# wasiahmad/context_attentive_ir

Measured on AMD Instinct MI355X. Metric: ranked (query,doc) pairs/sec, higher is better.
Workload: dtype f32; 1 GPU; cars, batch=16 sessions x session_len 7 x 10 candidates, q_len=4, doc_len=64, emb_dim=300, vocab=100000, f32, full-length Zipf ids; macro_batch=8, lanes=4, batches_in_flight=32, hipgraph=True, parallelism=single GPU, world_size=1

## Files before the change

### context_attentive_ir_amd/csrc/lstm_fold.hip

```cpp
#include <type_traits>
#include "split2.hpp"
#include <hip/hip_bf16.h>
#include <string>
#include <algorithm>

namespace nir {

int launch_linear(const float* a, int64_t lda, const int64_t* ids, const float* table, int E, int64_t rows_per_seq,
                  int64_t seq_stride, const float* w, int64_t ldw, const float* bias, const float* bias2, float* c,
                  int64_t ldc, int64_t M, int N, int K, int act, hipStream_t st);

__global__ void fold_permute_kernel(const float* __restrict__ wih, const float* __restrict__ bih, const float* __restrict__ bhh,
                                    int H, int ND, int E, float* __restrict__ wperm, float* __restrict__ bperm) {
    const int64_t i = (int64_t)blockIdx.x * blockDim.x + threadIdx.x;
    const int64_t rows = (int64_t)ND * 4 * H;
    if (i >= rows * E) return;
    const int64_t ro = i / E;
    const int k = (int)(i % E);
    const int gate = (int)(ro & 3), unit = (int)((ro >> 2) % H), dir = (int)((ro >> 2) / H);
    const int64_t ri = (int64_t)dir * 4 * H + (int64_t)gate * H + unit;
    wperm[i] = wih[ri * E + k];
    if (k == 0) bperm[ro] = bih[ri] + bhh[ri];
}

__global__ void iota_i64_kernel(int64_t* __restrict__ out, int64_t n) {
    const int64_t i = (int64_t)blockIdx.x * blockDim.x + threadIdx.x;
    if (i < n) out[i] = i;
}

int launch_fold_permute(const float* w_ih, const float* b_ih, const float* b_hh, int H, int ndir, int E, float* wperm, float* bperm, int64_t* iota, int64_t niota,
                        hipStream_t st) {
    const int64_t n = (int64_t)ndir * 4 * H * E;
    hipLaunchKernelGGL(fold_permute_kernel, dim3((unsigned)((n + 255) / 256)), dim3(256), 0, st, w_ih, b_ih, b_hh, H, ndir, E, wperm, bperm);
    if (iota && niota > 0) hipLaunchKernelGGL(iota_i64_kernel, dim3((unsigned)((niota + 255) / 256)), dim3(256), 0, st, iota, niota);
    NIR_CHECK_LAUNCH("fold_permute_kernel");
    return 0;
}

__global__ void f32_to_bf16_kernel(const float* __restrict__ src, unsigned short* __restrict__ dst, int64_t n) {
    const int64_t i = ((int64_t)blockIdx.x * blockDim.x + threadIdx.x) * 4;
    if (i + 3 < n) {
        const float4 v = *reinterpret_cast<const float4*>(src + i);
        ushort4 o;
        o.x = f2bf(v.x); o.y = f2bf(v.y); o.z = f2bf(v.z); o.w = f2bf(v.w);
        *reinterpret_cast<ushort4*>(dst + i) = o;
    } else {
        for (int64_t j = i; j < n; ++j) dst[j] = f2bf(src[j]);
    }
}

struct LstmPtArgs {
    const void* pt;
    const int64_t* ids;
    const int64_t* lens;
    const float* whh;
    float* out;
    int* err;
    int64_t M, V;
    int T, H, ND;
    int out_f16;
    const void* whh_frag;
    float* act;
    float* cst;
};

template <int G, int NT>
__global__ __launch_bounds__(1024) void lstm16_pt_kernel(LstmPtArgs p) {
    constexpr int SEQ = 16, KP = 16 * G, ZLD = KP + 4;
    constexpr uint32_t OOB = 0x7FFFFFF0u;
    extern __shared__ __attribute__((aligned(16))) float smem[];
    float* z = smem;
    int* lens_s = reinterpret_cast<int*>(z + 2 * SEQ * ZLD);
    int* ids_s = lens_s + SEQ;

    const int tid = threadIdx.x, lane = tid & 63, wave = tid >> 6;
    const int sq = lane & 15, kq = lane >> 4;
    const int dir = blockIdx.y;
    const int64_t m0 = (int64_t)blockIdx.x * SEQ;
    const int H = p.H, T = p.T, H4 = 4 * H;
    const int nvalid = (int)min((int64_t)SEQ, p.M - m0);
    const int OW = p.ND * H;
    const int64_t GW = (int64_t)p.ND * H4;
    const int ntiles = (H + 3) / 4;

    if (tid < SEQ) {
        int l = 0;
        if (tid < nvalid) {
            l = p.lens ? (int)p.lens[m0 + tid] : T;
            l = l < 0 ? 0 : (l > T ? T : l);
        }
        lens_s[tid] = l;
    }
    {
        bool bad = false;
        for (int e = tid; e < SEQ * T; e += 1024) {
            const int s = e / T;
            int64_t id = 0;
            if (s < nvalid) id = p.ids[m0 * T + e];
            if (id < 0 || id >= p.V) { bad = true; id = 0; }
            ids_s[e] = (int)id;
        }
        if (bad && p.err) atomicOr(p.err, 1);
    }
    for (int e = tid; e < 2 * SEQ * ZLD; e += 1024) z[e] = 0.f;
    __syncthreads();
    int tmax = 0;
#pragma unroll
    for (int s2 = 0; s2 < SEQ; ++s2) tmax = max(tmax, lens_s[s2]);
    const int mylen = lens_s[sq];

    float wreg[NT][4 * G];
    float creg[NT], hreg[NT];
    int unit_d[NT];
#pragma unroll
    for (int t = 0; t < NT; ++t) {
        const int tile = NT * wave + t;
        const int unit_a = 4 * tile + (sq >> 2), gate_a = sq & 3;
        const bool av = unit_a < H;
        const float* wr = p.whh + ((int64_t)dir * H4 + (int64_t)gate_a * H + (av ? unit_a : 0)) * H;
#pragma unroll
        for (int q = 0; q < G; ++q)
#pragma unroll
            for (int j = 0; j < 4; ++j) {
                const int k = 16 * q + 4 * kq + j;
                wreg[t][4 * q + j] = wr[k < H ? k : H - 1] * ((av && k < H) ? 1.f : 0.f);
            }
        unit_d[t] = 4 * tile + kq;
        creg[t] = 0.f;
        hreg[t] = 0.f;
    }
    const __amdgpu_buffer_rsrc_t out_rs = __builtin_amdgcn_make_buffer_rsrc(p.out + m0 * T * OW, 0,
                                                                             (int)((uint32_t)nvalid * T * OW * 4u), 0x00020000);
    const float* ptf = reinterpret_cast<const float*>(p.pt) + (int64_t)dir * H4;
    auto load_g = [&](int step, f32x4 (&dst)[NT]) {
        int s_ = min(step, mylen - 1);
        s_ = s_ < 0 ? 0 : s_;
        const int t_ = dir == 0 ? s_ : mylen - 1 - s_;
        const int id = ids_s[sq * T + (t_ < 0 ? 0 : t_)];
        const float* row = ptf + (int64_t)id * GW;
#pragma unroll
        for (int t = 0; t < NT; ++t) {
            const int u = unit_d[t] < H ? unit_d[t] : H - 1;
            dst[t] = *reinterpret_cast<const f32x4*>(row + 4 * u);
        }
    };
    f32x4 gcur[NT], gnext[NT];
    load_g(0, gcur);

    const bool has1 = NT * wave < ntiles;
    const bool has2 = NT > 1 && NT * wave + 1 < ntiles;
    for (int step = 0; step < tmax; ++step) {
        const float* zc = z + (step & 1) * SEQ * ZLD;
        float* zn = z + ((step + 1) & 1) * SEQ * ZLD;
        load_g(step + 1, gnext);
        const bool live = step < mylen;
        const int tt = dir == 0 ? step : mylen - 1 - step;
        auto cell_tile = [&](int t, const f32x4& acc) {
// ... 82 lines not shown
        const bool av = unit_a < H;
        const float* wr = p.whh + ((int64_t)dir * H4 + (int64_t)gate_a * H + (av ? unit_a : 0)) * H;
        const bool vec_ok = (H % 8) == 0 && ((reinterpret_cast<uintptr_t>(wr) & 15) == 0);
        if (vec_ok) {
#pragma unroll
            for (int kb = 0; kb < KB; ++kb) {
                const int k0 = 32 * kb + 8 * kq;
                const int kc = k0 + 8 <= H ? k0 : 0;
                const float4 a = *reinterpret_cast<const float4*>(wr + kc), b = *reinterpret_cast<const float4*>(wr + kc + 4);
                const float m = (av && k0 + 8 <= H) ? 1.f : 0.f;
                wreg[t][kb][0] = (_Float16)(a.x * m); wreg[t][kb][1] = (_Float16)(a.y * m);
                wreg[t][kb][2] = (_Float16)(a.z * m); wreg[t][kb][3] = (_Float16)(a.w * m);
                wreg[t][kb][4] = (_Float16)(b.x * m); wreg[t][kb][5] = (_Float16)(b.y * m);
                wreg[t][kb][6] = (_Float16)(b.z * m); wreg[t][kb][7] = (_Float16)(b.w * m);
                wbad |= !(fmaxf(fmaxf(fmaxf(fabsf(a.x), fabsf(a.y)), fmaxf(fabsf(a.z), fabsf(a.w))),
                                fmaxf(fmaxf(fabsf(b.x), fabsf(b.y)), fmaxf(fabsf(b.z), fabsf(b.w)))) * m < 65504.0f);
            }
        } else {
#pragma unroll
            for (int kb = 0; kb < KB; ++kb)
#pragma unroll
                for (int j = 0; j < 8; ++j) {
                    const int k = 32 * kb + 8 * kq + j;
                    const float w = wr[k < H ? k : H - 1] * ((av && k < H) ? 1.f : 0.f);
                    wreg[t][kb][j] = (_Float16)w;
                    wbad |= !(fabsf(w) < 65504.0f);
                }
        }
        unit_d[t] = 4 * tile + kq;
    }
    if (wbad && p.err) atomicOr(p.err, 2);
    for (int64_t mt = blockIdx.x; mt * SEQ < p.M; mt += gridDim.x) {
        __syncthreads();
        const int64_t m0 = mt * SEQ;
        const int nvalid = (int)min((int64_t)SEQ, p.M - m0);

        if (tid < SEQ) {
            int l = 0;
            if (tid < nvalid) {
                l = p.lens ? (int)p.lens[m0 + tid] : T;
                l = l < 0 ? 0 : (l > T ? T : l);
            }
            lens_s[tid] = l;
        }
        {
            bool bad = false;
            for (int e = tid; e < SEQ * T; e += 1024) {
                const int s = e / T;
                int64_t id = 0;
                if (s < nvalid) id = p.ids[m0 * T + e];
                if (id < 0 || id >= p.V) { bad = true; id = 0; }
                ids_s[e] = (int)id;
            }
            if (bad && p.err) atomicOr(p.err, 1);
        }
        for (int e = tid; e < SEQ * ZLD; e += 1024) reinterpret_cast<unsigned*>(z)[e] = 0u;
        __syncthreads();
        int tmax = 0;
#pragma unroll
        for (int s2 = 0; s2 < SEQ; ++s2) tmax = max(tmax, lens_s[s2]);
        const int mylen = lens_s[sq];

#pragma unroll
        for (int t = 0; t < NT; ++t) creg[t] = 0.f;
        const __amdgpu_buffer_rsrc_t out_rs =
            O16 ? __builtin_amdgcn_make_buffer_rsrc(reinterpret_cast<_Float16*>(p.out) + m0 * T * OW, 0, (int)((uint32_t)nvalid * T * OW * 2u), 0x00020000)
                : __builtin_amdgcn_make_buffer_rsrc(p.out + m0 * T * OW, 0, (int)((uint32_t)nvalid * T * OW * 4u), 0x00020000);
        const int wlen = __builtin_amdgcn_readfirstlane(lens_s[wave & (SEQ - 1)]);
        auto copy_out = [&](int s_, const unsigned short* zsrc) {
            const bool on = s_ >= 0 && s_ < wlen && 2 * lane < H;
            const int tt_ = dir == 0 ? s_ : wlen - 1 - s_;
            const uint32_t v = *reinterpret_cast<const uint32_t*>(zsrc + wave * ZLD + 2 * lane);
            const uint32_t off = on ? (uint32_t)((wave * T + tt_) * OW + dir * H + 2 * lane) * 2u : OOB;
            __builtin_amdgcn_raw_buffer_store_b32(v, out_rs, off, 0, 0);
        };
        const unsigned short* pth = reinterpret_cast<const unsigned short*>(p.pt) + (int64_t)dir * H4;
        auto id_of = [&](int step) {
            int s_ = min(step, mylen - 1);
            s_ = s_ < 0 ? 0 : s_;
            const int t_ = dir == 0 ? s_ : mylen - 1 - s_;
            return ids_s[sq * T + (t_ < 0 ? 0 : t_)];
        };
        auto load_g = [&](int id, uint2 (&dst)[NT]) {
            const unsigned short* row = pth + (int64_t)id * GW;
#pragma unroll
            for (int t = 0; t < NT; ++t) {
                const int u = unit_d[t] < H ? unit_d[t] : H - 1;
                dst[t] = *reinterpret_cast<const uint2*>(row + 4 * u);
            }
        };
        uint2 ga[NT], gb[NT];
        load_g(id_of(0), ga);
#pragma unroll
        for (int t = 0; t < (O16 ? 1 : NT); ++t) __builtin_amdgcn_raw_buffer_store_b32(0u, out_rs, OOB, 0, 0);
        load_g(id_of(1), gb);
#pragma unroll
        for (int t = 0; t < (O16 ? 1 : NT); ++t) __builtin_amdgcn_raw_buffer_store_b32(0u, out_rs, OOB, 0, 0);
        int id_n = id_of(2);

        for (int step = 0; step < tmax; ++step) {
            const unsigned short* zc = z + (step & 1) * SEQ * ZLD;
            unsigned short* zn = z + ((step + 1) & 1) * SEQ * ZLD;
            f32x4 acc[NT];
#pragma unroll
            for (int t = 0; t < NT; ++t) {
                asm volatile("" : "+v"(ga[t].x), "+v"(ga[t].y));
                acc[t] = (f32x4){bf2f((unsigned short)(ga[t].x & 0xFFFFu)), bf2f((unsigned short)(ga[t].x >> 16)),
                                 bf2f((unsigned short)(ga[t].y & 0xFFFFu)), bf2f((unsigned short)(ga[t].y >> 16))};
                ga[t] = gb[t];
            }
            const bool live = step < mylen;
            const int tt = dir == 0 ? step : mylen - 1 - step;
            const unsigned short* zr = zc + sq * ZLD + 8 * kq;
            if (O16) copy_out(step - 1, zc);
#pragma unroll
            for (int kb = 0; kb < KB; ++kb) {
                const f16x8 hb = *reinterpret_cast<const f16x8*>(zr + 32 * kb);
#pragma unroll
                for (int t = 0; t < NT; ++t) acc[t] = __builtin_amdgcn_mfma_f32_16x16x32_f16(wreg[t][kb], hb, acc[t], 0, 0, 0);
                if (kb == 0) {
                    load_g(id_n, gb);
                    id_n = id_of(step + 3);
                }
            }
#pragma unroll
            for (int t = 0; t < NT; ++t) {
                uint32_t off = OOB;
                float hv = 0.f;
                if (NT * wave + t < ntiles) {
                    const bool dv = unit_d[t] < H;
                    float hn;
                    lstm_cell_v(acc[t], creg[t], hn);
                    if (dv) reinterpret_cast<_Float16*>(zn)[sq * ZLD + unit_d[t]] = (_Float16)hn;
                    if (dv && live) off = (uint32_t)((sq * T + tt) * OW + dir * H + unit_d[t]) * 4u;
                    hv = hn;
                }
                if (!O16) __builtin_amdgcn_raw_buffer_store_b32(__float_as_uint(hv), out_rs, off, 0, 0);
            }
            lds_barrier();
        }
        if (O16 && tmax > 0) copy_out(tmax - 1, z + (tmax & 1) * SEQ * ZLD);
        for (int s_ = 0; s_ < nvalid; ++s_) {
            const int64_t ob = (m0 + s_) * T * OW + (int64_t)dir * H;
            for (int t2 = lens_s[s_] + wave; t2 < T; t2 += 16)
                for (int col = lane; col < H; col += 64) {
                    if (O16) reinterpret_cast<_Float16*>(p.out)[ob + (int64_t)t2 * OW + col] = (_Float16)0.f;
                    else p.out[ob + (int64_t)t2 * OW + col] = 0.f;
                }
        }
    }
}


#ifdef NIR_PT_TRACE
__device__ unsigned long long* g_pt_trace_dev;
#define PT_T(var) asm volatile("s_memtime %0\n\ts_waitcnt lgkmcnt(0)" : "=s"(var) :: "memory")
#endif
template <int KB, int NT, int NW, bool H1 = false, bool TR = false>
__global__ __launch_bounds__(64 * NW, NW <= 4 ? 2 : 1) void lstm16_pt_h2_kernel(LstmPtArgs p) {
    static_assert(!TR || !H1, "train-mode stores go with the fp32 output");
    constexpr int NTH = 64 * NW;
    constexpr int SEQ = 16, KP = 32 * KB, ZLD = KP + 8;
    constexpr uint32_t OOB = 0x7FFFFFF0u;
    constexpr bool SWZ = KB == 4;
    constexpr int KBS = SWZ ? 16 : 32;
    auto zoff = [](int s_, int k_) -> int {
        if constexpr (SWZ) {
            const int q_ = (k_ >> 3) & 3, b_ = k_ >> 5;
            return (s_ ^ (8 * (q_ & 1))) * ZLD + (8 * (q_ & 1) + 2 * b_ + (q_ >> 1)) * 8 + (k_ & 7);
        } else {
            return s_ * ZLD + k_;
        }
    };
#ifdef NIR_X_NOPIPE
    constexpr bool PIPE = false;
#else
    constexpr bool PIPE = NT >= 4 && NW == 8;
#endif
    constexpr bool DEFER = NW >= 8;
    const int TP = p.T + 3;
    extern __shared__ __attribute__((aligned(16))) float smem[];
    _Float16* z = reinterpret_cast<_Float16*>(smem);
    int* lens_s = reinterpret_cast<int*>(z + 4 * SEQ * ZLD);
    int* simd_s = lens_s + SEQ;
    int* ids_s = simd_s + 16;

    const int tid = threadIdx.x, lane = tid & 63, wave = tid >> 6;
    const int sq = lane & 15, kq = lane >> 4;
    const int dir = blockIdx.y;
    const int64_t m0 = (int64_t)blockIdx.x * SEQ;
    const int H = p.H, T = p.T, H4 = 4 * H;
    const int nvalid = (int)min((int64_t)SEQ, p.M - m0);
    const int OW = p.ND * H;
    const int64_t GW = (int64_t)p.ND * H4;
    f16x8 w1[NT][KB], w2[NT][KB];
    const bool use_frag = KB == 4 && NT == 4 && NW == 8 && p.whh_frag != nullptr && H == 128;
    if (use_frag) {
        const f16x8* fp = reinterpret_cast<const f16x8*>(p.whh_frag) + ((size_t)(dir * NW + wave) * NT * KB * 2) * 64 + lane;
#pragma unroll
        for (int t = 0; t < NT; ++t)
#pragma unroll
            for (int kb = 0; kb < KB; ++kb) {
                w1[t][kb] = fp[((t * KB + kb) * 2 + 0) * 64];
                w2[t][kb] = fp[((t * KB + kb) * 2 + 1) * 64];
            }
    }
    if (NW > 4 && lane == 0) simd_s[wave] = (int)__builtin_amdgcn_s_getreg(4 | (4 << 6) | (1 << 11));
    if (tid < SEQ) {
        int l = 0;
        if (tid < nvalid) {
            l = p.lens ? (int)p.lens[m0 + tid] : T;
            l = l < 0 ? 0 : (l > T ? T : l);
        }
        lens_s[tid] = l;
    }
    lds_barrier();
    {
        bool bad = false;
        for (int e = tid; e < SEQ * TP; e += NTH) {
            const int s_ = e / TP, k = e - s_ * TP;
            int64_t id = 0;
            if (s_ < nvalid) {
                const int l = lens_s[s_];
                int kk = k < l - 1 ? k : l - 1;
                kk = kk < 0 ? 0 : kk;
                int t_ = dir == 0 ? kk : l - 1 - kk;
                t_ = t_ < 0 ? 0 : t_;
                id = p.ids[(m0 + s_) * T + t_];
                if (k < T) {
                    const int64_t raw = p.ids[(m0 + s_) * T + k];
                    bad |= raw < 0 || raw >= p.V;
                }
            }
            if (id < 0 || id >= p.V) id = 0;
            ids_s[e] = (int)id;
        }
        if (bad && p.err) atomicOr(p.err, 1);
    }
    for (int e = tid; e < 2 * SEQ * ZLD; e += NTH) reinterpret_cast<unsigned*>(z)[e] = 0u;
    lds_barrier();
    int tmax = 0;
#pragma unroll
    for (int s2 = 0; s2 < SEQ; ++s2) tmax = max(tmax, lens_s[s2]);
    const int mylen = lens_s[sq];
    if (NW > 4) {
        const int mine = simd_s[wave];
        int rank = 0;
#pragma unroll
        for (int w2_ = 0; w2_ < NW; ++w2_) rank += (w2_ < wave && simd_s[w2_] == mine) ? 1 : 0;
        rank = __builtin_amdgcn_readfirstlane(rank);
        if (rank == 0) __builtin_amdgcn_s_setprio(3);
        else if (rank == 1) __builtin_amdgcn_s_setprio(2);
        else if (rank == 2) __builtin_amdgcn_s_setprio(1);
        else __builtin_amdgcn_s_setprio(0);
    }

    float creg[NT];
    const int u0 = NT * (4 * wave + kq);
    const bool wave_on = PIPE || NT * 4 * wave < H;
    const bool full = u0 + NT <= H;
    bool wbad = false;
#pragma unroll
    for (int t = 0; t < NT; ++t) {
        if (use_frag) { creg[t] = 0.f; continue; }
        const int unit_a = NT * (4 * wave + (sq >> 2)) + t, gate_a = sq & 3;
        const bool av = unit_a < H;
        const float* wr = p.whh + ((int64_t)dir * H4 + (int64_t)gate_a * H + (av ? unit_a : 0)) * H;
        float wv[KB][8];
        const bool vec_ok = (H % 8) == 0 && ((reinterpret_cast<uintptr_t>(wr) & 15) == 0);
        if (vec_ok) {
#pragma unroll
            for (int kb = 0; kb < KB; ++kb) {
                const int k0 = 32 * kb + 8 * kq;
                const int kc = k0 + 8 <= H ? k0 : 0;
                const float4 a = *reinterpret_cast<const float4*>(wr + kc), b = *reinterpret_cast<const float4*>(wr + kc + 4);
                const float m = (av && k0 + 8 <= H) ? 1.f : 0.f;
                wv[kb][0] = a.x * m; wv[kb][1] = a.y * m; wv[kb][2] = a.z * m; wv[kb][3] = a.w * m;
                wv[kb][4] = b.x * m; wv[kb][5] = b.y * m; wv[kb][6] = b.z * m; wv[kb][7] = b.w * m;
            }
        } else {
#pragma unroll
            for (int kb = 0; kb < KB; ++kb)
#pragma unroll
                for (int j = 0; j < 8; ++j) {
                    const int k = 32 * kb + 8 * kq + j;
                    wv[kb][j] = wr[k < H ? k : H - 1] * ((av && k < H) ? 1.f : 0.f);
                }
        }
#pragma unroll
        for (int kb = 0; kb < KB; ++kb)
#pragma unroll
            for (int j = 0; j < 8; ++j) {
                const float w = wv[kb][j];
                const _Float16 a = split2_hi1_rne(w);
                w1[t][kb][j] = a;
                w2[t][kb][j] = split2_lo1(w, a);
                wbad |= !(fabsf(w) < 32768.0f);
            }
        creg[t] = 0.f;
    }
    if (wbad && p.err) atomicOr(p.err, 2);
    const __amdgpu_buffer_rsrc_t out_rs = H1 ? __builtin_amdgcn_make_buffer_rsrc(reinterpret_cast<_Float16*>(p.out) + m0 * T * OW, 0,
                                                                                  (int)((uint32_t)nvalid * T * OW * 2u), 0x00020000)
                                             : __builtin_amdgcn_make_buffer_rsrc(p.out + m0 * T * OW, 0, (int)((uint32_t)nvalid * T * OW * 4u), 0x00020000);
    const __amdgpu_buffer_rsrc_t act_rs = __builtin_amdgcn_make_buffer_rsrc(TR ? p.act + m0 * T * GW : p.out, 0,
                                                                             TR ? (int)((uint32_t)nvalid * T * (uint32_t)GW * 4u) : 0, 0x00020000);
    const __amdgpu_buffer_rsrc_t cst_rs = __builtin_amdgcn_make_buffer_rsrc(TR ? p.cst + m0 * T * OW : p.out, 0,
                                                                             TR ? (int)((uint32_t)nvalid * T * OW * 4u) : 0, 0x00020000);
    const float* ptf = reinterpret_cast<const float*>(p.pt) + (int64_t)dir * H4;
    const float* pb[NT];
#pragma unroll
    for (int t = 0; t < NT; ++t) pb[t] = ptf + 4 * (u0 + t < H ? u0 + t : H - 1);
    const uint32_t gw = (uint32_t)GW;
    auto load_g = [&](int id, f32x4 (&dst)[NT]) {
#ifdef NIR_X_NOROWS
        return;
#endif
        const uint64_t ro = (uint64_t)(uint32_t)id * gw;
#pragma unroll
        for (int t = 0; t < NT; ++t) dst[t] = *reinterpret_cast<const f32x4*>(pb[t] + ro);
    };
    f32x4 gnext[NT];
    uint32_t hprev[NT];
#pragma unroll
    for (int t = 0; t < NT; ++t) hprev[t] = 0u;
    const bool split = NT == 4 && p.out_f16 == 2;
    uint32_t poff = OOB;
    auto store_prev = [&]() {
#ifdef NIR_X_NOSTORE
        return;
#endif
        if (H1) {
            __builtin_amdgcn_raw_buffer_store_b64((u32x2){hprev[0], hprev[1 % NT]}, out_rs, poff == OOB ? OOB : poff >> 1, 0, 0);
            return;
        }
        if (NT == 4) {
            __builtin_amdgcn_raw_buffer_store_b128((u32x4){hprev[0], hprev[1 % NT], hprev[2 % NT], hprev[3 % NT]}, out_rs, full ? poff : OOB, 0, 0);
        } else if (NT == 2) {
            __builtin_amdgcn_raw_buffer_store_b64((u32x2){hprev[0], hprev[1 % NT]}, out_rs, full ? poff : OOB, 0, 0);
        }
        if ((NT != 4 && NT != 2) || !full) {
#pragma unroll
            for (int t = 0; t < NT; ++t)
                __builtin_amdgcn_raw_buffer_store_b32(hprev[t], out_rs, (u0 + t < H && poff != OOB) ? poff + 4u * t : OOB, 0, 0);
        }
    };
    const int* idp = ids_s + sq * TP;
    load_g(idp[0], gnext);
    int id_n = idp[1];
    uint32_t soff = (uint32_t)(((sq * T + (dir == 0 ? 0 : mylen - 1)) * OW + dir * H + u0) * 4);
    const uint32_t sstep = (uint32_t)(dir == 0 ? OW * 4 : -(OW * 4));
    f32x4 acc[NT], acx[NT];
    float hn[NT] = {};
#ifdef NIR_X_NOGATES
    auto gates = [&](int t) { hn[t] = (acx[t][0] + acc[t][1]) * 1e-3f; };
#else
    float tga[TR ? NT : 1][4];
    auto gates = [&](int t) {
        if constexpr (TR) {
            const f32x4 x = split2_combine(acc[t], acx[t]);
            const float gi = fast_sigmoid(x[0]), gf = fast_sigmoid(x[1]), gg = fast_tanh(x[2]), go = fast_sigmoid(x[3]);
            const float cn = gf * creg[t] + gi * gg;
            creg[t] = cn;
            hn[t] = go * fast_tanh(cn);
            tga[t][0] = gi; tga[t][1] = gf; tga[t][2] = gg; tga[t][3] = go;
        } else {
            lstm_cell_v(split2_combine(acc[t], acx[t]), creg[t], hn[t]);
        }
    };
    uint32_t aoff = (uint32_t)(((int64_t)(sq * T + (dir == 0 ? 0 : mylen - 1)) * GW + dir * H4 + u0) * 4);
    const uint32_t astep = (uint32_t)(dir == 0 ? GW * 4 : -(GW * 4));
#endif
#ifdef NIR_PT_TRACE
    unsigned long long tr_a = 0, tr_b = 0, tr_c = 0, tr_t0 = 0, tr_t1 = 0, tr_t2 = 0, tr_first = 0, tr_l = 0, tr_m = 0;
#endif
    for (int step = 0; step < tmax; ++step) {
#ifdef NIR_PT_TRACE
        { unsigned long long tn; PT_T(tn); if (step > 0) tr_c += tn - tr_t2; else tr_first = tn; tr_t0 = tn; }
#endif
        const _Float16* zc = z + (step & 1) * 2 * SEQ * ZLD;
        _Float16* zn = z + ((step + 1) & 1) * 2 * SEQ * ZLD;
#pragma unroll
        for (int t = 0; t < NT; ++t) {
            acc[t] = gnext[t];
            acx[t] = (f32x4){0.f, 0.f, 0.f, 0.f};
        }
        const bool live = step < mylen;
        const _Float16* zr = zc + zoff(sq, 8 * kq);
        if (!wave_on) {
#ifdef NIR_X_BURST
        } else if constexpr (NT == 4 && NW == 8) {
            f16x8 hh1[KB], hh2[KB];
#pragma unroll
            for (int kb = 0; kb < KB; ++kb) {
                hh1[kb] = *reinterpret_cast<const f16x8*>(zr + KBS * kb);
                hh2[kb] = *reinterpret_cast<const f16x8*>(zr + SEQ * ZLD + KBS * kb);
            }
#pragma unroll
            for (int kb = 0; kb < KB; ++kb) {
#pragma unroll
                for (int t = 0; t < NT; ++t) acc[t] = __builtin_amdgcn_mfma_f32_16x16x32_f16(w1[t][kb], hh1[kb], acc[t], 0, 0, 0);
#pragma unroll
                for (int t = 0; t < NT; ++t) acx[t] = __builtin_amdgcn_mfma_f32_16x16x32_f16(w1[t][kb], hh2[kb], acx[t], 0, 0, 0);
#pragma unroll
                for (int t = 0; t < NT; ++t) acx[t] = __builtin_amdgcn_mfma_f32_16x16x32_f16(w2[t][kb], hh1[kb], acx[t], 0, 0, 0);
                if (kb == 0) {
                    if (DEFER) store_prev();
                    load_g(id_n, gnext);
                    id_n = idp[step + 2];
                }
            }
#ifdef NIR_PT_TRACE
#pragma unroll
            for (int t = 0; t < NT; ++t) asm volatile("" : "+v"(acc[t]), "+v"(acx[t]));
            PT_T(tr_t1); tr_a += tr_t1 - tr_t0;
#endif
#pragma unroll
            for (int t = 0; t < NT; ++t) gates(t);
#endif
        } else if constexpr (!PIPE) {
#pragma unroll
            for (int kb = 0; kb < KB; ++kb) {
                const f16x8 h1 = *reinterpret_cast<const f16x8*>(zr + KBS * kb);
                const f16x8 h2 = *reinterpret_cast<const f16x8*>(zr + SEQ * ZLD + KBS * kb);
#pragma unroll
                for (int t = 0; t < NT; ++t) {
                    acc[t] = __builtin_amdgcn_mfma_f32_16x16x32_f16(w1[t][kb], h1, acc[t], 0, 0, 0);
                    acx[t] = __builtin_amdgcn_mfma_f32_16x16x32_f16(w1[t][kb], h2, acx[t], 0, 0, 0);
                    acx[t] = __builtin_amdgcn_mfma_f32_16x16x32_f16(w2[t][kb], h1, acx[t], 0, 0, 0);
                }
                if (kb == 0) {
                    if (DEFER) store_prev();
                    load_g(id_n, gnext);
                    id_n = idp[step + 2];
                }
            }
#ifdef NIR_PT_TRACE
#pragma unroll
            for (int t = 0; t < NT; ++t) asm volatile("" : "+v"(acc[t]), "+v"(acx[t]));
            PT_T(tr_t1); tr_a += tr_t1 - tr_t0;
#endif
#pragma unroll
            for (int t = 0; t < NT; ++t) gates(t);
        } else {
            f16x8 hh1[KB], hh2[H1 ? 1 : KB];
#pragma unroll
            for (int kb = 0; kb < KB; ++kb) {
                hh1[kb] = *reinterpret_cast<const f16x8*>(zr + KBS * kb);
                if (!H1) hh2[H1 ? 0 : kb] = *reinterpret_cast<const f16x8*>(zr + SEQ * ZLD + KBS * kb);
            }
#ifdef NIR_PT_TRACE
            { unsigned long long tn; PT_T(tn); tr_l += tn - tr_t0; }
#endif
#pragma unroll
            for (int t = 0; t < NT; ++t) {
#pragma unroll
                for (int kb = 0; kb < KB; ++kb) {
                    acc[t] = __builtin_amdgcn_mfma_f32_16x16x32_f16(w1[t][kb], hh1[kb], acc[t], 0, 0, 0);
                    if (!H1) acx[t] = __builtin_amdgcn_mfma_f32_16x16x32_f16(w1[t][kb], hh2[H1 ? 0 : kb], acx[t], 0, 0, 0);
                    acx[t] = __builtin_amdgcn_mfma_f32_16x16x32_f16(w2[t][kb], hh1[kb], acx[t], 0, 0, 0);
                }
                if (t == 0) {
                    if (DEFER) store_prev();
                    load_g(id_n, gnext);
                    id_n = idp[step + 2];
                } else {
#ifdef NIR_PT_TRACE
                    if (t == 1) { asm volatile("" : "+v"(acc[0]), "+v"(acx[0])); unsigned long long tn; PT_T(tn); tr_m += tn - tr_t0; }
#endif
                    gates(t - 1);
#pragma unroll
                    for (int q = 0; q < (H1 ? 2 : 3) * KB; ++q) {
                        __builtin_amdgcn_sched_group_barrier(0x008, 1, 0);
                        __builtin_amdgcn_sched_group_barrier(0x002, 3, 0);
                    }
                }
            }
#ifdef NIR_PT_TRACE
            asm volatile("" : "+v"(acc[NT - 1]), "+v"(acx[NT - 1]));
            PT_T(tr_t1); tr_a += tr_t1 - tr_t0;
#endif
            gates(NT - 1);
        }
        if (full && (NT == 4 || NT == 2)) {
            _Float16 a[NT], r[NT];
#pragma unroll
            for (int t = 0; t < NT; ++t) a[t] = split2_hi1_rne(hn[t]);
            {
                _Float16 as_[NT];
#pragma unroll
                for (int t = 0; t < NT; t += 2) {
                    const f16x2 p2 = (f16x2){a[t], a[(t + 1) % NT]} * (f16x2){(_Float16)SPLIT2_SCALE, (_Float16)SPLIT2_SCALE};
                    as_[t] = p2[0]; as_[(t + 1) % NT] = p2[1];
                }
#pragma unroll
                for (int t = 0; t < NT; ++t) r[t] = (_Float16)__builtin_fmaf(hn[t], SPLIT2_SCALE, -(float)as_[t]);
            }
            if (NT == 4) {
                const f16x4 av = (f16x4){a[0], a[1 % NT], a[2 % NT], a[3 % NT]}, rv = (f16x4){r[0], r[1 % NT], r[2 % NT], r[3 % NT]};
                *reinterpret_cast<f16x4*>(zn + zoff(sq, u0)) = av;
                if (!H1) *reinterpret_cast<f16x4*>(zn + SEQ * ZLD + zoff(sq, u0)) = rv;
                if (H1) {
                    const u32x2 au = __builtin_bit_cast(u32x2, av);
                    hprev[0] = au[0]; hprev[1 % NT] = au[1];
                } else
                if (split) {
                    const u32x2 au = __builtin_bit_cast(u32x2, av), ru = __builtin_bit_cast(u32x2, rv);
                    hprev[0] = au[0]; hprev[1 % NT] = au[1]; hprev[2 % NT] = ru[0]; hprev[3 % NT] = ru[1];
                }
            } else {
                *reinterpret_cast<f16x2*>(zn + zoff(sq, u0)) = (f16x2){a[0], a[1 % NT]};
                *reinterpret_cast<f16x2*>(zn + SEQ * ZLD + zoff(sq, u0)) = (f16x2){r[0], r[1 % NT]};
            }
        } else {
#pragma unroll
            for (int t = 0; t < NT; ++t)
                if (u0 + t < H) {
                    const _Float16 a = split2_hi1_rne(hn[t]);
                    zn[zoff(sq, u0 + t)] = a;
                    zn[SEQ * ZLD + zoff(sq, u0 + t)] = split2_lo1(hn[t], a);
                }
        }
        if (!split && !H1) {
#pragma unroll
            for (int t = 0; t < NT; ++t) hprev[t] = __float_as_uint(hn[t]);
        }
        poff = live ? soff : OOB;
        soff += sstep;
#ifndef NIR_X_NOGATES
        if constexpr (TR) {
            const uint32_t ao = live ? aoff : OOB;
            if (NT == 4 && full) {
#pragma unroll
                for (int r = 0; r < 4; ++r)
                    __builtin_amdgcn_raw_buffer_store_b128((u32x4){__float_as_uint(tga[0][r]), __float_as_uint(tga[1 % NT][r]), __float_as_uint(tga[2 % NT][r]),
                                                                   __float_as_uint(tga[3 % NT][r])}, act_rs, ao == OOB ? OOB : ao + (uint32_t)(r * H * 4), 0, 0);
                __builtin_amdgcn_raw_buffer_store_b128((u32x4){__float_as_uint(creg[0]), __float_as_uint(creg[1 % NT]), __float_as_uint(creg[2 % NT]),
                                                               __float_as_uint(creg[3 % NT])}, cst_rs, poff, 0, 0);
            } else if (NT == 2 && full) {
#pragma unroll
                for (int r = 0; r < 4; ++r)
                    __builtin_amdgcn_raw_buffer_store_b64((u32x2){__float_as_uint(tga[0][r]), __float_as_uint(tga[1 % NT][r])}, act_rs,
                                                          ao == OOB ? OOB : ao + (uint32_t)(r * H * 4), 0, 0);
                __builtin_amdgcn_raw_buffer_store_b64((u32x2){__float_as_uint(creg[0]), __float_as_uint(creg[1 % NT])}, cst_rs, poff, 0, 0);
            } else {
#pragma unroll
                for (int t = 0; t < NT; ++t) {
                    const bool uv = u0 + t < H && ao != OOB;
#pragma unroll
                    for (int r = 0; r < 4; ++r)
                        __builtin_amdgcn_raw_buffer_store_b32(__float_as_uint(tga[t][r]), act_rs, uv ? ao + (uint32_t)((r * H + t) * 4) : OOB, 0, 0);
                    __builtin_amdgcn_raw_buffer_store_b32(__float_as_uint(creg[t]), cst_rs, uv ? poff + 4u * t : OOB, 0, 0);
                }
            }
            aoff += astep;
        }
#endif
        if (!DEFER) store_prev();
#ifdef NIR_PT_TRACE
        PT_T(tr_t2); tr_b += tr_t2 - tr_t1;
#endif
        lds_barrier();
    }
    if (DEFER) store_prev();
#ifdef NIR_PT_TRACE
    if (blockIdx.x == 0 && blockIdx.y == 0 && lane == 0 && g_pt_trace_dev) {
        unsigned long long tn; PT_T(tn);
        unsigned long long* o = g_pt_trace_dev + wave * 8;
        o[0] = tr_a; o[1] = tr_b; o[2] = tr_c; o[3] = tn - tr_first; o[4] = __builtin_amdgcn_s_getreg(4 | (0 << 6) | (15 << 11)); o[5] = tmax; o[6] = tr_l; o[7] = tr_m;
    }
#endif
    for (int s_ = 0; s_ < nvalid; ++s_) {
        if (H1) {
            _Float16* orow = reinterpret_cast<_Float16*>(p.out) + (m0 + s_) * T * OW + (int64_t)dir * H;
            for (int t2 = lens_s[s_] + wave; t2 < T; t2 += NW)
                for (int col = lane; col < H; col += 64) orow[(int64_t)t2 * OW + col] = (_Float16)0.f;
            continue;
        }
        float* orow = p.out + (m0 + s_) * T * OW + (int64_t)dir * H;
        for (int t2 = lens_s[s_] + wave; t2 < T; t2 += NW)
            for (int col = lane; col < H; col += 64) orow[(int64_t)t2 * OW + col] = 0.f;
    }
}

template <int KB, int NT, int NW = 16, bool H1 = false, bool TR = false>
static int launch_pt_h2(const LstmPtArgs& p, hipStream_t st) {
    static const std::string pname = "lstm16_pt_h2_kernel<" + std::to_string(KB) + "," + std::to_string(NT) + (NW == 16 ? "" : "," + std::to_string(NW)) + (TR ? ",false,true" : H1 ? ",true" : "") + ">";
    const size_t lds = (size_t)(4 * 16 * (32 * KB + 8)) * 2 + 2 * 16 * 4 + (size_t)16 * (p.T + 3) * 4;
    ProfScope ps(prof_shape_name(pname.c_str(), (long long)p.M, p.T, p.H), st);
#ifdef NIR_PT_TRACE
    { unsigned long long* d = g_debug_buf; (void)hipMemcpyToSymbolAsync(HIP_SYMBOL(g_pt_trace_dev), &d, sizeof(d), 0, hipMemcpyHostToDevice, st); }
#endif
    hipLaunchKernelGGL((lstm16_pt_h2_kernel<KB, NT, NW, H1, TR>), dim3((unsigned)((p.M + 15) / 16), (unsigned)p.ND), dim3(64 * NW), lds, st, p);
    NIR_CHECK_LAUNCH("nir_bilstm_folded_fwd[f16x2]");
    return 0;
}

template <int G, int NT>
static int launch_pt(const LstmPtArgs& p, hipStream_t st) {
    static const std::string pname = "lstm16_pt_kernel<" + std::to_string(G) + "," + std::to_string(NT) + ">";
    const size_t lds = (size_t)(2 * 16 * (16 * G + 4)) * 4 + 16 * 4 + (size_t)16 * p.T * 4;
    ProfScope ps(prof_shape_name(pname.c_str(), (long long)p.M, p.T, p.H), st);
    hipLaunchKernelGGL((lstm16_pt_kernel<G, NT>), dim3((unsigned)((p.M + 15) / 16), (unsigned)p.ND), dim3(1024), lds, st, p);
    NIR_CHECK_LAUNCH("nir_bilstm_folded_fwd[f32]");
    return 0;
}
static int cu_count() {
    static const int ncu = [] {
        int dev = 0;
        hipDeviceProp_t prop;
        return (hipGetDevice(&dev) == hipSuccess && hipGetDeviceProperties(&prop, dev) == hipSuccess && prop.multiProcessorCount > 0)
                   ? prop.multiProcessorCount : 256;
    }();
    return ncu;
}

template <bool O16>
__global__ __launch_bounds__(512, 4) void lstm16_pt_bf16w8_kernel(LstmPtArgs p) {
    constexpr int KB = 4, NT = 4, NW = 8, NTH = 64 * NW, SEQ = 16, KP = 32 * KB, ZLD = KP + 8;
    constexpr uint32_t OOB = 0x7FFFFFF0u;
    extern __shared__ __attribute__((aligned(16))) float smem[];
    unsigned short* z = reinterpret_cast<unsigned short*>(smem);
    f16x8* wl = reinterpret_cast<f16x8*>(z + 2 * SEQ * ZLD);
    int* lens_s = reinterpret_cast<int*>(wl + NW * NT * 64);
    int* ids_s = lens_s + SEQ;
    const int tid = threadIdx.x, lane = tid & 63, wave = tid >> 6;
    const int sq = lane & 15, kq = lane >> 4;
    const int dir = blockIdx.y;
    const int H = p.H, T = p.T, H4 = 4 * H, TP = p.T + 4;
    const int OW = p.ND * H;
    const int64_t GW = (int64_t)p.ND * H4;
    const int u0 = NT * (4 * wave + kq);
    const bool full = u0 + NT <= H;

    f16x8 wreg[NT][KB - 1];
    bool wbad = false;
#pragma unroll
    for (int t = 0; t < NT; ++t) {
        const int unit_a = NT * (4 * wave + (sq >> 2)) + t, gate_a = sq & 3;
        const bool av = unit_a < H;
        const float* wr = p.whh + ((int64_t)dir * H4 + (int64_t)gate_a * H + (av ? unit_a : 0)) * H;
        const bool vec_ok = (H % 8) == 0 && ((reinterpret_cast<uintptr_t>(wr) & 15) == 0);
#pragma unroll
        for (int kb = 0; kb < KB; ++kb) {
            float wv[8];
            const int k0 = 32 * kb + 8 * kq;
            if (vec_ok) {
                const int kc = k0 + 8 <= H ? k0 : 0;
                const float4 a = *reinterpret_cast<const float4*>(wr + kc), b = *reinterpret_cast<const float4*>(wr + kc + 4);
                const float m = (av && k0 + 8 <= H) ? 1.f : 0.f;
                wv[0] = a.x * m; wv[1] = a.y * m; wv[2] = a.z * m; wv[3] = a.w * m; wv[4] = b.x * m; wv[5] = b.y * m; wv[6] = b.z * m; wv[7] = b.w * m;
            } else {
#pragma unroll
                for (int j = 0; j < 8; ++j) wv[j] = wr[k0 + j < H ? k0 + j : H - 1] * ((av && k0 + j < H) ? 1.f : 0.f);
            }
            f16x8 wf;
#pragma unroll
            for (int j = 0; j < 8; ++j) {
                wf[j] = (_Float16)wv[j];
                wbad |= !(fabsf(wv[j]) < 65504.0f);
            }
            if (kb < KB - 1) wreg[t][kb < KB - 1 ? kb : 0] = wf;
            else wl[(wave * NT + t) * 64 + lane] = wf;
        }
    }
    if (wbad && p.err) atomicOr(p.err, 2);
    const f16x8* wlp = wl + wave * NT * 64 + lane;
    const unsigned short* pth = reinterpret_cast<const unsigned short*>(p.pt) + (int64_t)dir * H4;
    const unsigned short* pb = pth + 4 * (full ? u0 : 0);
    const uint32_t gw = (uint32_t)GW;

    for (int64_t mt = blockIdx.x; mt * SEQ < p.M; mt += gridDim.x) {
        __syncthreads();
        const int64_t m0 = mt * SEQ;
        const int nvalid = (int)min((int64_t)SEQ, p.M - m0);
        if (tid < SEQ) {
            int l = 0;
            if (tid < nvalid) {
                l = p.lens ? (int)p.lens[m0 + tid] : T;
                l = l < 0 ? 0 : (l > T ? T : l);
            }
            lens_s[tid] = l;
        }
        __syncthreads();
        {
            bool bad = false;
            for (int e = tid; e < SEQ * TP; e += NTH) {
                const int s_ = e / TP, k = e - s_ * TP;
                int64_t id = 0;
                if (s_ < nvalid) {
                    const int l = lens_s[s_];
                    int kk = k < l - 1 ? k : l - 1;
                    kk = kk < 0 ? 0 : kk;
                    int t_ = dir == 0 ? kk : l - 1 - kk;
                    t_ = t_ < 0 ? 0 : t_;
                    id = p.ids[(m0 + s_) * T + t_];
                    if (k < T) {
                        const int64_t raw = p.ids[(m0 + s_) * T + k];
                        bad |= raw < 0 || raw >= p.V;
                    }
                }
                if (id < 0 || id >= p.V) id = 0;
                ids_s[e] = (int)id;
            }
            if (bad && p.err) atomicOr(p.err, 1);
        }
        for (int e = tid; e < SEQ * ZLD; e += NTH) reinterpret_cast<unsigned*>(z)[e] = 0u;
        __syncthreads();
        int tmax = 0;
#pragma unroll
        for (int s2 = 0; s2 < SEQ; ++s2) tmax = max(tmax, lens_s[s2]);
        const int mylen = lens_s[sq];
        float creg[NT];
#pragma unroll
        for (int t = 0; t < NT; ++t) creg[t] = 0.f;
        const __amdgpu_buffer_rsrc_t out_rs =
            O16 ? __builtin_amdgcn_make_buffer_rsrc(reinterpret_cast<_Float16*>(p.out) + m0 * T * OW, 0, (int)((uint32_t)nvalid * T * OW * 2u), 0x00020000)
                : __builtin_amdgcn_make_buffer_rsrc(p.out + m0 * T * OW, 0, (int)((uint32_t)nvalid * T * OW * 4u), 0x00020000);
        int wlen[2];
#pragma unroll
        for (int r = 0; r < 2; ++r) wlen[r] = __builtin_amdgcn_readfirstlane(lens_s[2 * wave + r]);
        auto copy_out = [&](int s_, const unsigned short* zsrc) {
#pragma unroll
            for (int r = 0; r < 2; ++r) {
                const int sr = 2 * wave + r;
                const bool on = s_ >= 0 && s_ < wlen[r] && 2 * lane < H;
                const int tt_ = dir == 0 ? s_ : wlen[r] - 1 - s_;
                const uint32_t v = *reinterpret_cast<const uint32_t*>(zsrc + sr * ZLD + 2 * lane);
                __builtin_amdgcn_raw_buffer_store_b32(v, out_rs, on ? (uint32_t)((sr * T + tt_) * OW + dir * H + 2 * lane) * 2u : OOB, 0, 0);
            }
        };
        const int* idp = ids_s + sq * TP;
        auto load_g = [&](int id, uint4 (&dst)[2]) {
            const uint4* row = reinterpret_cast<const uint4*>(pb + (uint64_t)(uint32_t)id * gw);
            dst[0] = row[0];
            dst[1] = row[1];
        };
        uint4 ga[2];
        load_g(idp[0], ga);
        int id_n = idp[1];
        float hprev[NT] = {0.f, 0.f, 0.f, 0.f};
        uint32_t poff = OOB;
        uint32_t soff = (uint32_t)(((sq * T + (dir == 0 ? 0 : mylen - 1)) * OW + dir * H + u0) * 4);
        const uint32_t sstep = (uint32_t)(dir == 0 ? OW * 4 : -(OW * 4));
        auto store_prev = [&]() {
            __builtin_amdgcn_raw_buffer_store_b128((u32x4){__float_as_uint(hprev[0]), __float_as_uint(hprev[1]), __float_as_uint(hprev[2]), __float_as_uint(hprev[3])},
// ... 274 lines not shown
```

Measured before the change: 8.326 million pairs/s.

## Make folded BiLSTM kernel persistent with prefetch of next group's ids and lengths

For the 8-wave variant, the grid is capped at about one block per CU per direction, and each block loops over several 16-sequence groups. While the current group's recurrence runs, the block prefetches the next group's token ids and lengths into extra LDS buffers and then builds the gather indices. The aim is to remove per-block launch and setup cost and to hide the id and length loads behind the MFMA loop. In exchange it uses more LDS, adds register pressure, and may lower occupancy or parallelism when there are only a few groups.

Result: no change. 8.290 million pairs/s (-0.4%).

```diff
diff --git a/context_attentive_ir_amd/csrc/lstm_fold.hip b/context_attentive_ir_amd/csrc/lstm_fold.hip
--- a/context_attentive_ir_amd/csrc/lstm_fold.hip
+++ b/context_attentive_ir_amd/csrc/lstm_fold.hip
@@ -3,6 +3,7 @@
 #include <hip/hip_bf16.h>
 #include <string>
 #include <algorithm>
+#include <mutex>
 
 namespace nir {
 
@@ -391,7 +392,7 @@
 }
 
 
-#ifdef NIR_PT_TRACE
+#if defined(NIR_PT_TRACE) || defined(NIR_PT_LIFE)
 __device__ unsigned long long* g_pt_trace_dev;
 #define PT_T(var) asm volatile("s_memtime %0\n\ts_waitcnt lgkmcnt(0)" : "=s"(var) :: "memory")
 #endif
@@ -427,9 +428,16 @@
     const int tid = threadIdx.x, lane = tid & 63, wave = tid >> 6;
     const int sq = lane & 15, kq = lane >> 4;
     const int dir = blockIdx.y;
-    const int64_t m0 = (int64_t)blockIdx.x * SEQ;
+#ifdef NIR_PT_LIFE
+    unsigned long long lf_start, lf_t = 0, lf_loop = 0, lf_ng = 0, lf_first = 0, lf_a = 0, lf_b = 0, lf_c = 0, lf_d = 0, lf_m = 0;
+    PT_T(lf_start);
+#endif
     const int H = p.H, T = p.T, H4 = 4 * H;
-    const int nvalid = (int)min((int64_t)SEQ, p.M - m0);
+    const int64_t ngroups = (p.M + SEQ - 1) / SEQ, gstride = gridDim.x;
+    const bool multi = gstride < ngroups;
+    int* pos_x = ids_s + SEQ * TP;
+    int* lens_x = pos_x + SEQ * T;
+    auto lens_of = [&](int r) -> int* { return r == 0 ? lens_s : lens_x + SEQ * (r - 1); };
     const int OW = p.ND * H;
     const int64_t GW = (int64_t)p.ND * H4;
     f16x8 w1[NT][KB], w2[NT][KB];
@@ -445,43 +453,61 @@
             }
     }
     if (NW > 4 && lane == 0) simd_s[wave] = (int)__builtin_amdgcn_s_getreg(4 | (4 << 6) | (1 << 11));
-    if (tid < SEQ) {
+    auto load_len = [&](int64_t g_) -> int {
+        const int64_t m_ = g_ * SEQ + tid;
         int l = 0;
-        if (tid < nvalid) {
-            l = p.lens ? (int)p.lens[m0 + tid] : T;
+        if (tid < SEQ && g_ < ngroups && m_ < p.M) {
+            l = p.lens ? (int)p.lens[m_] : T;
             l = l < 0 ? 0 : (l > T ? T : l);
         }
-        lens_s[tid] = l;
-    }
-    lds_barrier();
-    {
+        return l;
+    };
+    auto stage_lens = [&](int* dst, int64_t g_) {
+        const int l = load_len(g_);
+        if (tid < SEQ) dst[tid] = l;
+    };
+    auto stage_ids = [&](int* dst, const int* lens_g, int64_t g_) {
+        const int64_t mg = g_ * SEQ;
+        const int nv = (int)min((int64_t)SEQ, p.M - mg);
         bool bad = false;
-        for (int e = tid; e < SEQ * TP; e += NTH) {
-            const int s_ = e / TP, k = e - s_ * TP;
-            int64_t id = 0;
-            if (s_ < nvalid) {
-                const int l = lens_s[s_];
+        constexpr int UN = 3;
+        for (int e0 = tid; e0 < SEQ * TP; e0 += UN * NTH) {
+            int64_t idv[UN], raw[UN];
+            bool in[UN], chk[UN];
+#pragma unroll
+            for (int u = 0; u < UN; ++u) {
+                const int e = min(e0 + u * NTH, SEQ * TP - 1);
+                const int s_ = e / TP, k = e - s_ * TP;
+                in[u] = s_ < nv;
+                chk[u] = in[u] && k < T;
+                const int sc = min(s_, nv - 1);
+                const int l = lens_g[sc];
                 int kk = k < l - 1 ? k : l - 1;
                 kk = kk < 0 ? 0 : kk;
                 int t_ = dir == 0 ? kk : l - 1 - kk;
                 t_ = t_ < 0 ? 0 : t_;
-                id = p.ids[(m0 + s_) * T + t_];
-                if (k < T) {
-                    const int64_t raw = p.ids[(m0 + s_) * T + k];
-                    bad |= raw < 0 || raw >= p.V;
-                }
-            }
-            if (id < 0 || id >= p.V) id = 0;
-            ids_s[e] = (int)id;
+                idv[u] = p.ids[(mg + sc) * T + t_];
+                raw[u] = p.ids[(mg + sc) * T + min(k, T - 1)];
+            }
+#pragma unroll
+            for (int u = 0; u < UN; ++u) {
+                const int e = e0 + u * NTH;
+                bad |= chk[u] && (raw[u] < 0 || raw[u] >= p.V);
+                const int64_t id = (in[u] && idv[u] >= 0 && idv[u] < p.V) ? idv[u] : 0;
+                if (e < SEQ * TP) dst[e] = (int)id;
+            }
         }
         if (bad && p.err) atomicOr(p.err, 1);
-    }
-    for (int e = tid; e < 2 * SEQ * ZLD; e += NTH) reinterpret_cast<unsigned*>(z)[e] = 0u;
+    };
+    auto zero_h = [&]() {
+        for (int e = tid; e < 2 * SEQ * ZLD; e += NTH) reinterpret_cast<unsigned*>(z)[e] = 0u;
+    };
+    stage_lens(lens_s, blockIdx.x);
+    if (multi) stage_lens(lens_of(1), blockIdx.x + gstride);
     lds_barrier();
-    int tmax = 0;
-#pragma unroll
-    for (int s2 = 0; s2 < SEQ; ++s2) tmax = max(tmax, lens_s[s2]);
-    const int mylen = lens_s[sq];
+    stage_ids(ids_s, lens_s, blockIdx.x);
+    zero_h();
+    lds_barrier();
     if (NW > 4) {
         const int mine = simd_s[wave];
         int rank = 0;
@@ -501,7 +527,7 @@
     bool wbad = false;
 #pragma unroll
     for (int t = 0; t < NT; ++t) {
-        if (use_frag) { creg[t] = 0.f; continue; }
+        if (use_frag) continue;
         const int unit_a = NT * (4 * wave + (sq >> 2)) + t, gate_a = sq & 3;
         const bool av = unit_a < H;
         const float* wr = p.whh + ((int64_t)dir * H4 + (int64_t)gate_a * H + (av ? unit_a : 0)) * H;
@@ -536,9 +562,41 @@
                 w2[t][kb][j] = split2_lo1(w, a);
                 wbad |= !(fabsf(w) < 32768.0f);
             }
-        creg[t] = 0.f;
     }
     if (wbad && p.err) atomicOr(p.err, 2);
+    const float* ptf = reinterpret_cast<const float*>(p.pt) + (int64_t)dir * H4;
+    const float* pb[NT];
+#pragma unroll
+    for (int t = 0; t < NT; ++t) pb[t] = ptf + 4 * (u0 + t < H ? u0 + t : H - 1);
+    const uint32_t gw = (uint32_t)GW;
+    const bool split = NT == 4 && p.out_f16 == 2;
+    const uint32_t sstep = (uint32_t)(dir == 0 ? OW * 4 : -(OW * 4));
+    auto load_g = [&](int id, f32x4 (&dst)[NT]) {
+#ifdef NIR_X_NOROWS
+        return;
+#endif
+        const uint64_t ro = (uint64_t)(uint32_t)id * gw;
+#pragma unroll
+        for (int t = 0; t < NT; ++t) dst[t] = *reinterpret_cast<const f32x4*>(pb[t] + ro);
+    };
+    f32x4 gnext[NT];
+    load_g(ids_s[sq * TP], gnext);
+    int lr = 0;
+    bool sbad = false;
+    for (int64_t g = blockIdx.x;; g += gstride) {
+#ifdef NIR_PT_LIFE
+    if (lf_ng > 0) { unsigned long long tn; PT_T(tn); lf_b += tn - lf_m; lf_m = tn; }
+#endif
+    const int64_t m0 = g * SEQ;
+    const int nvalid = (int)min((int64_t)SEQ, p.M - m0);
+    const int* lens_c = lens_of(lr);
+    const bool more = g + gstride < ngroups;
+    int tmax = 0;
+#pragma unroll
+    for (int s2 = 0; s2 < SEQ; ++s2) tmax = max(tmax, lens_c[s2]);
+    const int mylen = lens_c[sq];
+#pragma unroll
+    for (int t = 0; t < NT; ++t) creg[t] = 0.f;
     const __amdgpu_buffer_rsrc_t out_rs = H1 ? __builtin_amdgcn_make_buffer_rsrc(reinterpret_cast<_Float16*>(p.out) + m0 * T * OW, 0,
                                                                                   (int)((uint32_t)nvalid * T * OW * 2u), 0x00020000)
                                              : __builtin_amdgcn_make_buffer_rsrc(p.out + m0 * T * OW, 0, (int)((uint32_t)nvalid * T * OW * 4u), 0x00020000);
@@ -546,24 +604,9 @@
                                                                              TR ? (int)((uint32_t)nvalid * T * (uint32_t)GW * 4u) : 0, 0x00020000);
     const __amdgpu_buffer_rsrc_t cst_rs = __builtin_amdgcn_make_buffer_rsrc(TR ? p.cst + m0 * T * OW : p.out, 0,
                                                                              TR ? (int)((uint32_t)nvalid * T * OW * 4u) : 0, 0x00020000);
-    const float* ptf = reinterpret_cast<const float*>(p.pt) + (int64_t)dir * H4;
-    const float* pb[NT];
-#pragma unroll
-    for (int t = 0; t < NT; ++t) pb[t] = ptf + 4 * (u0 + t < H ? u0 + t : H - 1);
-    const uint32_t gw = (uint32_t)GW;
-    auto load_g = [&](int id, f32x4 (&dst)[NT]) {
-#ifdef NIR_X_NOROWS
-        return;
-#endif
-        const uint64_t ro = (uint64_t)(uint32_t)id * gw;
-#pragma unroll
-        for (int t = 0; t < NT; ++t) dst[t] = *reinterpret_cast<const f32x4*>(pb[t] + ro);
-    };
-    f32x4 gnext[NT];
     uint32_t hprev[NT];
 #pragma unroll
     for (int t = 0; t < NT; ++t) hprev[t] = 0u;
-    const bool split = NT == 4 && p.out_f16 == 2;
     uint32_t poff = OOB;
     auto store_prev = [&]() {
 #ifdef NIR_X_NOSTORE
@@ -585,10 +628,28 @@
         }
     };
     const int* idp = ids_s + sq * TP;
-    load_g(idp[0], gnext);
     int id_n = idp[1];
+#ifdef NIR_PT_LIFE
+    if (lf_ng > 0) { unsigned long long tn; PT_T(tn); lf_c += tn - lf_m; lf_m = tn; }
+#endif
+    const int64_t mgn = (g + gstride) * SEQ;
+    const int nvn = more ? (int)min((int64_t)SEQ, p.M - mgn) : 0, npos = nvn * T;
+    const int nst = more ? (SEQ * T + NTH - 1) / NTH : 0;
+    int s_iss = 0, s_wr = 0, slen = 0;
+    int64_t sraw = 0;
+    auto st_issue = [&]() {
+        sraw = p.ids[mgn * T + min(s_iss * NTH + tid, npos - 1)];
+        if (s_iss == 0) slen = load_len(g + 2 * gstride);
+        ++s_iss;
+    };
+    auto st_write = [&]() {
+        const int e = s_wr * NTH + tid;
+        const bool oob = sraw < 0 || sraw >= p.V;
+        sbad |= e < npos && oob;
+        if (e < SEQ * T) pos_x[e] = (e < npos && !oob) ? (int)sraw : 0;
+        ++s_wr;
+    };
     uint32_t soff = (uint32_t)(((sq * T + (dir == 0 ? 0 : mylen - 1)) * OW + dir * H + u0) * 4);
-    const uint32_t sstep = (uint32_t)(dir == 0 ? OW * 4 : -(OW * 4));
     f32x4 acc[NT], acx[NT];
     float hn[NT] = {};
 #ifdef NIR_X_NOGATES
@@ -613,6 +674,10 @@
 #ifdef NIR_PT_TRACE
     unsigned long long tr_a = 0, tr_b = 0, tr_c = 0, tr_t0 = 0, tr_t1 = 0, tr_t2 = 0, tr_first = 0, tr_l = 0, tr_m = 0;
 #endif
+#ifdef NIR_PT_LIFE
+    PT_T(lf_t);
+    if (lf_ng == 0) lf_first = lf_t - lf_start; else lf_d += lf_t - lf_m;
+#endif
     for (int step = 0; step < tmax; ++step) {
 #ifdef NIR_PT_TRACE
         { unsigned long long tn; PT_T(tn); if (step > 0) tr_c += tn - tr_t2; else tr_first = tn; tr_t0 = tn; }
@@ -624,6 +689,7 @@
             acc[t] = gnext[t];
             acx[t] = (f32x4){0.f, 0.f, 0.f, 0.f};
         }
+        if (!TR && s_wr < s_iss) st_write();
         const bool live = step < mylen;
         const _Float16* zr = zc + zoff(sq, 8 * kq);
         if (!wave_on) {
@@ -700,6 +766,7 @@
                     acx[t] = __builtin_amdgcn_mfma_f32_16x16x32_f16(w2[t][kb], hh1[kb], acx[t], 0, 0, 0);
                 }
                 if (t == 0) {
+                    if (!TR && s_iss < nst) st_issue();
                     if (DEFER) store_prev();
                     load_g(id_n, gnext);
                     id_n = idp[step + 2];
@@ -801,36 +868,98 @@
 #endif
         lds_barrier();
     }
+#ifdef NIR_PT_LIFE
+    { unsigned long long tn; PT_T(tn); lf_loop += tn - lf_t; ++lf_ng; lf_m = tn; }
+#endif
+    int idn0 = 0;
+    if (more) {
+        const bool late = s_wr < nst;
+        if (s_wr < s_iss) st_write();
+        while (s_iss < nst) { st_issue(); st_write(); }
+        if (late) lds_barrier();
+        const int* lens_n = lens_of(lr == 2 ? 0 : lr + 1);
+        for (int e = tid; e < SEQ * TP; e += NTH) {
+            const int s_ = e / TP, k = e - s_ * TP;
+            const int l = lens_n[s_];
+            int kk = k < l - 1 ? k : l - 1;
+            kk = kk < 0 ? 0 : kk;
+            int t_ = dir == 0 ? kk : l - 1 - kk;
+            t_ = t_ < 0 ? 0 : t_;
+            ids_s[e] = s_ < nvn ? pos_x[s_ * T + t_] : 0;
+        }
+        const int ln = lens_n[sq];
+        idn0 = sq < nvn ? pos_x[sq * T + ((dir == 0 || ln < 1) ? 0 : ln - 1)] : 0;
+    }
+    for (int s_ = 0; s_ < nvalid; ++s_) {
+        const int ls = __builtin_amdgcn_readlane(mylen, s_);
+        if (H1) {
+            _Float16* orow = reinterpret_cast<_Float16*>(p.out) + (m0 + s_) * T * OW + (int64_t)dir * H;
+            for (int t2 = ls + wave; t2 < T; t2 += NW)
+                for (int col = lane; col < H; col += 64) orow[(int64_t)t2 * OW + col] = (_Float16)0.f;
+            continue;
+        }
+        float* orow = p.out + (m0 + s_) * T * OW + (int64_t)dir * H;
+        for (int t2 = ls + wave; t2 < T; t2 += NW)
+            for (int col = lane; col < H; col += 64) orow[(int64_t)t2 * OW + col] = 0.f;
+    }
     if (DEFER) store_prev();
 #ifdef NIR_PT_TRACE
+    if (g == 0 && blockIdx.y == 0 && lane == 0 && g_pt_trace_dev) {
+        unsigned long long tn; PT_T(tn);
+        unsigned long long* o = g_pt_trace_dev + wave * 8;
+        o[0] = tr_a; o[1] = tr_b; o[2] = tr_c; o[3] = tn - tr_first; o[4] = __builtin_amdgcn_s_getreg(4 | (0 << 6) | (15 << 11)); o[5] = tmax; o[6] = tr_l; o[7] = tr_m;
+    }
+#endif
+#ifdef NIR_PT_LIFE
+    { unsigned long long tn; PT_T(tn); lf_a += tn - lf_m; lf_m = tn; }
+#endif
+    if (!more) break;
+    load_g(idn0, gnext);
+    zero_h();
+    if (tid < SEQ) lens_of(lr == 0 ? 2 : lr - 1)[tid] = slen;
+    lds_barrier();
+    lr = lr == 2 ? 0 : lr + 1;
+    }
+    if (sbad && p.err) atomicOr(p.err, 1);
+#ifdef NIR_PT_LIFE
     if (blockIdx.x == 0 && blockIdx.y == 0 && lane == 0 && g_pt_trace_dev) {
         unsigned long long tn; PT_T(tn);
         unsigned long long* o = g_pt_trace_dev + wave * 8;
-        o[0] = tr_a; o[1] = tr_b; o[2] = tr_c; o[3] = tn - tr_first; o[4] = __builtin_amdgcn_s_getreg(4 | (0 << 6) | (15 << 11)); o[5] = tmax; o[6] = tr_l; o[7] = tr_m;
-    }
-#endif
-    for (int s_ = 0; s_ < nvalid; ++s_) {
-        if (H1) {
-            _Float16* orow = reinterpret_cast<_Float16*>(p.out) + (m0 + s_) * T * OW + (int64_t)dir * H;
-            for (int t2 = lens_s[s_] + wave; t2 < T; t2 += NW)
-                for (int col = lane; col < H; col += 64) orow[(int64_t)t2 * OW + col] = (_Float16)0.f;
-            continue;
-        }
-        float* orow = p.out + (m0 + s_) * T * OW + (int64_t)dir * H;
-        for (int t2 = lens_s[s_] + wave; t2 < T; t2 += NW)
-            for (int col = lane; col < H; col += 64) orow[(int64_t)t2 * OW + col] = 0.f;
-    }
-}
+        o[0] = tn - lf_start; o[1] = lf_loop; o[2] = lf_ng; o[3] = lf_first; o[4] = lf_a; o[5] = 0; o[6] = lf_b; o[7] = lf_c + (lf_d << 32);
+    }
+#endif
+}
+
+static int cu_count();
 
 template <int KB, int NT, int NW = 16, bool H1 = false, bool TR = false>
 static int launch_pt_h2(const LstmPtArgs& p, hipStream_t st) {
     static const std::string pname = "lstm16_pt_h2_kernel<" + std::to_string(KB) + "," + std::to_string(NT) + (NW == 16 ? "" : "," + std::to_string(NW)) + (TR ? ",false,true" : H1 ? ",true" : "") + ">";
-    const size_t lds = (size_t)(4 * 16 * (32 * KB + 8)) * 2 + 2 * 16 * 4 + (size_t)16 * (p.T + 3) * 4;
+    auto lds_bytes = [](int T, bool multi) {
+        return (size_t)(4 * 16 * (32 * KB + 8)) * 2 + 2 * 16 * 4 + (size_t)16 * (T + 3) * 4 + (multi ? (size_t)16 * T * 4 + 2 * 16 * 4 : 0);
+    };
+    const int64_t groups = (p.M + 15) / 16;
+    int64_t gx = groups;
+    if (NW == 8) {
+#ifdef NIR_X_RESCAP78
+        gx = std::min(groups, (int64_t)std::max(1, (cu_count() * 7 / 8 + p.ND - 1) / p.ND));
+#elif !defined(NIR_X_NORES)
+        gx = std::min(groups, (int64_t)std::max(1, (cu_count() + p.ND - 1) / p.ND));
+#endif
+    }
+    const bool multi = gx < groups;
+    const size_t lds = lds_bytes(p.T, multi);
+    if (multi) {
+        static std::once_flag once;
+        std::call_once(once, [&] {
+            (void)hipFuncSetAttribute((const void*)lstm16_pt_h2_kernel<KB, NT, NW, H1, TR>, hipFuncAttributeMaxDynamicSharedMemorySize, (int)lds_bytes(512, true));
+        });
+    }
     ProfScope ps(prof_shape_name(pname.c_str(), (long long)p.M, p.T, p.H), st);
-#ifdef NIR_PT_TRACE
+#if defined(NIR_PT_TRACE) || defined(NIR_PT_LIFE)
     { unsigned long long* d = g_debug_buf; (void)hipMemcpyToSymbolAsync(HIP_SYMBOL(g_pt_trace_dev), &d, sizeof(d), 0, hipMemcpyHostToDevice, st); }
 #endif
-    hipLaunchKernelGGL((lstm16_pt_h2_kernel<KB, NT, NW, H1, TR>), dim3((unsigned)((p.M + 15) / 16), (unsigned)p.ND), dim3(64 * NW), lds, st, p);
+    hipLaunchKernelGGL((lstm16_pt_h2_kernel<KB, NT, NW, H1, TR>), dim3((unsigned)gx, (unsigned)p.ND), dim3(64 * NW), lds, st, p);
     NIR_CHECK_LAUNCH("nir_bilstm_folded_fwd[f16x2]");
     return 0;
 }
```
